# nucypher/TFHE.jl

Hardware: AMD Instinct MI355X
Metric: bootstrapped gates/sec (whole node), N=1024 (higher is better)
Workload: dtype int32 torus / f64 transform; 1 GPU; batch of 4096 independent gate_nand() bootstraps per GPU, tfhe_parameters_80 (n=500, N=1024, k=1, l=2, Bg=2^10, ks t=8, base 2^2); inputs=resident in HBM, launch=one process

## Files before the change

### tfhe.jl_amd/csrc/engine.hpp

```cpp
#pragma once
#include <hip/hip_runtime.h>

#include <algorithm>
#include <atomic>
#include <cstdarg>
#include <cstdio>
#include <cstring>
#include <new>
#include <string>
#include <thread>
#include <vector>

#include "../../include/tfhe_mi355x.h"
#include "experiment.hpp"
#include "br_core.hpp"

using namespace tfhe;

#include "kernels_blind_rotate.hpp"
#include "kernels_anyn.hpp"
#include "kernels_n512.hpp"
#include "kernels_keyswitch.hpp"

struct ErrBuf {
    char s[512] = {0};
    const char *c_str() const { return s; }
    void set(const char *msg) { snprintf(s, sizeof s, "%s", msg ? msg : ""); }
    ErrBuf &operator=(const char *msg) { set(msg); return *this; }
    void format(const char *fmt, ...) __attribute__((format(printf, 2, 3)))
    {
        va_list ap;
        va_start(ap, fmt);
        vsnprintf(s, sizeof s, fmt, ap);
        va_end(ap);
    }
};
extern thread_local ErrBuf g_create_error;

struct DevBuf {
    void *p = nullptr;
    size_t cap = 0;
    hipError_t reserve(size_t bytes)
    {
        if (bytes <= cap) return hipSuccess;
        if (p) (void)hipFree(p);
        p = nullptr; cap = 0;
        size_t want = bytes + bytes / 4 + 256;
        hipError_t e = hipMalloc(&p, want);
        if (e == hipSuccess) cap = want;
        return e;
    }
    void release() { if (p) (void)hipFree(p); p = nullptr; cap = 0; }
};

struct PairXfer {
    static constexpr int kSlots = 4;
    struct Slot {
        DevBuf out, idx_src;
        DevBuf in, idx_dst;
        int32_t *h_idx = nullptr; size_t h_idx_cap = 0;
        void *h_rows = nullptr; size_t h_rows_cap = 0;
        hipEvent_t ready = nullptr;
        hipEvent_t taken = nullptr;
        bool pending = false;
    } slot[kSlots];
    unsigned next = 0;
};

struct KsKey {
    int mode = 0;
    int parties = 1;
    int kN = 0;
    void *p = nullptr;
    size_t per_party = 0;
    int stride = 0;
    int wtiles = 0;
};
inline void release(KsKey &k)
{
    if (k.p) (void)hipFree(k.p);
    k = KsKey{};
}

struct tfhe_ctx {
    tfhe_params P{};
    int device = 0;
    ErrBuf err;
    std::vector<tfhe_ctx *> kids;
    std::vector<uint8_t> kid_ran;

    hipStream_t stream = nullptr;
    static constexpr int kTimingSlots = 33;
    hipEvent_t evring[kTimingSlots][4] = {};
    hipEvent_t *ev = evring[0];
    int64_t timed_calls = 0;
    hipEvent_t done_ev = nullptr;
    bool done_pending = false;
    bool timing_valid = false;
    bool own_pending = false;
    int64_t last_rotations = 0;
    std::string last_kernel;
    int ks_slices_large = 2;
    int ks_variant = 4;
    int64_t br_small = 1024;
    int br_prio_pct = 90;
    int br_general = 0;
    int br_split = 1;
    int timing_events = 1;
    int br_rt_l = 0;
    int64_t br_tiny = -2;

    cplx *d_tables = nullptr;
    Tables T{};
    Gadget g{};
    cplx *d_anyn_tab = nullptr;
    int br_anyn = 0;
    int anyn_spec = -1;
    bool anyn() const
    {
        if (br_anyn) return true;
        if (P.parties > 1) return P.N != kN || P.parties > 8 || P.bs_l > 8;
        if (n512()) return false;
        return (P.N != kN && P.N != 2048) || P.k > 4;
    }
    bool n512() const { return !br_anyn && P.parties == 1 && P.N == 512 && P.k == 1; }

    cplx *d_bk = nullptr;       size_t bk_polys = 0;
    KsKey ks;
    bool have_bk = false;
    bool have_ks() const { return ks.mode != 0 && ks.parties == 1; }
    cplx *d_mk_bk = nullptr;
    int mk_parties = 0;
    bool have_mk_bk = false;
    bool have_mk_ks() const { return ks.mode != 0 && ks.parties > 1; }

    int32_t *d_wires = nullptr; int64_t num_wires = 0;
    int wires_parties = 0;
    size_t wire_words() const { return wires_parties ? (size_t)wires_parties * P.n + 1 : (size_t)P.n + 1; }

    DevBuf bara, ext, map, io[4], diag, abar, mk_acc, spec;
    DevBuf tv, tv_index;
    DevBuf tv_bodies, tv_ext;
    cplx *d_tgsw = nullptr;        int64_t tgsw_count = 0;
    DevBuf lvl_ws[2], lvl_data, lvl_spec;
    cplx *d_mk_tgsw = nullptr;     int64_t mk_tgsw_count = 0;
    int32_t *d_mk_tgsw_party = nullptr;
    size_t diag_rows = 0;
    bool mk_force_general = false;
    int n2048_rw = 0;
    int mkg_rw = 0;
    int mkg_variant = 0;
    int mkg_acc = -1;
    int mk_rw = 0;
    bool measure_margin = false;
    int exact_domain = 2;
    double exact_bound_log2 = 0;
    double exact_margin = 0;
    tfhe_ctx *twin = nullptr;
    std::atomic<hipStream_t> twin_stream{nullptr};
    bool borrows_keys = false;
    bool slot_busy[2] = {false, false};
    std::atomic<std::thread::id> submit_thread{};
    uint32_t submits = 0;
    std::vector<std::vector<uint8_t>> wire_valid;
    std::vector<int32_t> wire_owner;
    std::vector<uint8_t> peer_ok;
    std::vector<struct PairXfer *> xfer;
    int level_exchange = 0;
    int64_t level_split_min = 4096;
    std::vector<int32_t> kid_tickets[2];
    int cu_count = 256;
    int w2_rw = 0;
    int n512_w2 = -1;
    int n512_rw = 0;
    int k2_w3 = -1;
    int k2_rw = 0;
    int v3_rw = 0;
    int64_t pipeline_min = 4096;
    bool last_call_two_streams = false;
    struct MapStage { void *h = nullptr; size_t cap = 0; hipEvent_t ev = nullptr; bool pending = false; };
    static constexpr int kMapStages = 4;
    MapStage map_stage[kMapStages];
    unsigned map_next = 0;
    MapStage *map_cur = &map_stage[0];
    void *h_map = nullptr;
// ... 200 lines not shown
```

### tfhe.jl_amd/csrc/engine_dispatch.hip

```cpp
#define TFHE_EMIT_KEYSWITCH_KERNELS
#include "engine.hpp"
#include "br_launch.hpp"

#include <map>
#include <mutex>
#include <functional>

int32_t ensure_dyn_lds(tfhe_ctx *c, const void *fn, size_t bytes, const char *what)
{
    static std::mutex mu;
    static std::map<std::pair<int, const void *>, size_t> have;
    std::lock_guard<std::mutex> lk(mu);
    size_t &cur = have[std::make_pair(c->device, fn)];
    if (cur >= bytes) return TFHE_OK;
    const hipError_t e = hipFuncSetAttribute(fn, hipFuncAttributeMaxDynamicSharedMemorySize, (int)bytes);
    if (e != hipSuccess) return c->set_err(TFHE_ERR_DEVICE, "hipFuncSetAttribute(%s, %zu bytes of LDS) failed: %s", what, bytes, hipGetErrorString(e));
    cur = bytes;
    return TFHE_OK;
}

int32_t prepare_diag(tfhe_ctx *c, size_t R, hipStream_t s, DiagArgs &d)
{
    d.margin_bits = nullptr; d.clk = nullptr; d.phase = nullptr;
    c->diag_rows = 0;
// ... 190 lines not shown
            if (best[i - n] + kK2RoundCost[n] < best[i]) { best[i] = best[i - n] + kK2RoundCost[n]; take[i] = n; }
    int tail = 0;
    double total = best[q];
    for (int t = 1; allow_w3 && t <= 2 && (size_t)t <= q; t++)
        if (best[q - t] + kK2W3RoundCost[t] < total) { total = best[q - t] + kK2W3RoundCost[t]; tail = t; }
    std::vector<int> rounds;
    for (size_t i = q - (size_t)tail; i > 0; i -= (size_t)take[i]) rounds.push_back(take[i]);
    std::sort(rounds.begin(), rounds.end(), std::greater<int>());
    std::vector<K2Seg> seg;
    size_t done = 0;
    for (size_t i = 0; i < rounds.size() && done < R;) {
        size_t j = i;
        while (j < rounds.size() && rounds[j] == rounds[i]) j++;
        const size_t want = (size_t)rounds[i] * (j - i) * cus;
        if ((j == rounds.size() && !tail) || done + want >= R) { seg.push_back({R - done, 0}); done = R; break; }
        seg.push_back({want, 0});
        done += want;
        i = j;
    }
    if (done < R) seg.push_back({R - done, 1});
    return seg;
}

int32_t launch_blind_rotate(tfhe_ctx *c, size_t R, int32_t mu, hipStream_t s, const TvPtrs *tv)
{
    if (tv && c->measure_margin) return c->set_err(TFHE_ERR_STATE, "bootstrap_tv: no DIAG instantiation of the TV kernels (measure_margin is on)");
    DiagArgs diag;
    int32_t rc = prepare_diag(c, R, s, diag);
    if (rc) return rc;
    alloc_checkpoint();
    std::vector<K2Seg> seg;
    const bool tuned_l = c->P.bs_l == 2 || c->P.bs_l == 3;
    if (c->anyn()) {
    } else if (c->br_split && !c->br_general && !c->measure_margin && c->P.N == kN && c->P.k == 2 && tuned_l && (c->k2_rw == 0 || c->k2_rw == 7) && c->k2_w3 != 1) {
        seg = k2_partition(R, (size_t)c->cu_count, c->k2_w3 < 0);
    } else if (c->br_split && !c->br_general && c->P.N == kN && c->P.k == 1 && c->br_small > 0) {
        const size_t resident = 8 * (size_t)c->cu_count;
        if (R > resident && R % resident > 0 && R % resident <= (size_t)c->br_small) seg = {{R - R % resident, -1}, {R % resident, -1}};
    }
    auto part = [&](size_t first, size_t count, int kind) {
        const int32_t r = launch_blind_rotate_part(c, first, count, mu, s, diag, kind, tv);
        if (!r && tv) c->last_kernel += "+tv";
        return r;
    };
    if (seg.empty()) return part(0, R, -1);
    if (seg.size() == 1) return part(0, R, seg[0].kind);
    std::string names;
    size_t first = 0;
    for (const K2Seg &sg : seg) {
        rc = part(first, sg.count, sg.kind);
        if (rc) return rc;
        if (names.empty() || names.substr(names.rfind(" + ") == std::string::npos ? 0 : names.rfind(" + ") + 3) != c->last_kernel)
            names += (names.empty() ? "" : " + ") + c->last_kernel;
        first += sg.count;
    }
    c->last_kernel = names;
    return TFHE_OK;
}

template <class A>
static A ks_args(const tfhe_ctx *c, const int32_t *e0, const int32_t *e1, const int32_t *dst, const int32_t *ext, int32_t *out)
{
    const int P = c->ks.parties, kN = c->ks.kN, n = c->P.n;
    A a{};
    a.ext = ext; a.e0 = e0; a.e1 = e1; a.dst = dst; a.out = out;
    a.n = n; a.kN = kN;
    a.in_stride = P * kN + 1; a.in_off = 0; a.in_b = P * kN; a.out_stride = P * n + 1; a.out_off = 0; a.out_b = P * n;
    return a;
}

int32_t launch_keyswitch(tfhe_ctx *c, size_t G, const int32_t *e0, const int32_t *e1, const int32_t *dst, const int32_t *ext, int32_t *out, hipStream_t s)
{
    const KsKey &K = c->ks;
    const int P = K.parties, kN = K.kN, n = c->P.n;
    if (K.mode == 4) {
        Ks4Args a = ks_args<Ks4Args>(c, e0, e1, dst, ext, out);
        a.G = (int)G; a.wtiles = K.wtiles;
        a.kslices = (P > 1 || kN % 512 != 0) ? 1 : (G <= 512 ? 16 : c->ks_slices_large);
        if (a.kslices > 1) {
            const Ks3Args i3 = ks_args<Ks3Args>(c, e0, e1, dst, ext, out);
            hipLaunchKernelGGL(ks3_init_kernel, dim3((unsigned)G), dim3(256), 0, s, i3);
        }
        a.Gpad = (int)((G + 63) / 64 * 64);
        HIP_TRY(c, c->abar.reserve((size_t)(kN / 4) * a.Gpad * 16));
        a.abar_t = (const i32x4 *)c->abar.p;
        for (int p = 0; p < P; p++) {
            a.in_off = p * kN; a.out_off = p * n; a.add_b = (p == 0);
            a.bmat = (const i32x4 *)K.p + (size_t)p * K.per_party;
            hipLaunchKernelGGL(ks4_digits_kernel, dim3((unsigned)(a.Gpad / 32), (unsigned)(kN / 128)), dim3(128), 0, s, a, (i32x4 *)c->abar.p);
            hipLaunchKernelGGL(keyswitch_kernel_v4, dim3((unsigned)((G + 255) / 256), (unsigned)K.wtiles, (unsigned)a.kslices), dim3(256), 0, s, a);
        }
    } else if (K.mode == 3) {
        Ks3Args a = ks_args<Ks3Args>(c, e0, e1, dst, ext, out);
        a.t = c->P.ks_t; a.log2_base = 2; a.stride = K.stride; a.G = (int)G;
        a.ksp = (const int32_t *)K.p;
        hipLaunchKernelGGL(ks3_init_kernel, dim3((unsigned)G), dim3(256), 0, s, a);
        const unsigned tiles = (unsigned)((G + KS3_G - 1) / KS3_G);
        for (int p = 0; p < P; p++) {
            a.in_off = p * kN; a.out_off = p * n;
            a.ksp = (const int32_t *)K.p + (size_t)p * K.per_party;
            hipLaunchKernelGGL(keyswitch_kernel_v3, dim3(tiles * KS3_SLICES, (unsigned)((K.stride + 511) / 512)), dim3(128), 0, s, a);
        }
    } else {
        KsArgs a = ks_args<KsArgs>(c, e0, e1, dst, ext, out);
        a.t = c->P.ks_t; a.log2_base = c->P.ks_log2_base;
        for (int p = 0; p < P; p++) {
            a.in_off = p * kN; a.out_off = p * n; a.add_b = (p == 0);
            a.ks = (const int32_t *)K.p + (size_t)p * K.per_party;
            hipLaunchKernelGGL(keyswitch_kernel, dim3((unsigned)G, (unsigned)((n + 1 + 256 * KS1_WPT - 1) / (256 * KS1_WPT))), dim3(256), 0, s, a);
        }
    }
    HIP_TRY(c, hipGetLastError());
    return TFHE_OK;
}
```

### tfhe.jl_amd/csrc/engine_keys.hip

```cpp
#define TFHE_EMIT_KEYPREP_KERNELS
#include "engine.hpp"
#include "kernels_keygen.hpp"

static int32_t check_key_source(tfhe_ctx *c, const void *p, const char *who)
{
    hipPointerAttribute_t at;
    const hipError_t e = hipPointerGetAttributes(&at, p);
    if (e != hipSuccess) { (void)hipGetLastError(); return TFHE_OK; }
    if (at.type == hipMemoryTypeDevice && at.device != c->device)
        return c->set_err(TFHE_ERR_DEVICE, "%s: the key buffer lives on device %d, this context on device %d: pass a host copy (peer access between GPUs is not assumed)",
                          who, at.device, c->device);
    return TFHE_OK;
}

void quiesce(tfhe_ctx *c)
{
    if (c->stream) (void)hipStreamSynchronize(c->stream);
    if (c->done_pending) { (void)hipEventSynchronize(c->done_ev); c->done_pending = false; }
    c->own_pending = false;
    if (c->twin && c->twin->stream) (void)hipStreamSynchronize(c->twin->stream);
    c->slot_busy[0] = c->slot_busy[1] = false;
    if (c->twin) {
        tfhe_ctx *t = c->twin;
        t->d_bk = nullptr; t->have_bk = false; t->ks = KsKey{};
// ... 39 lines not shown
        if (big && is_c128)
            hipLaunchKernelGGL(bk_permute_c128_kernel_n2048, dim3((unsigned)npolys), dim3(128), 0, c->stream, (const cplx *)d_in, c->d_bk);
        else if (big)
            hipLaunchKernelGGL(bk_prepare_kernel_n2048, dim3((unsigned)npolys), dim3(128), 0, c->stream, (const int32_t *)d_in, c->d_bk,
                               (const cplx *)(c->d_tables + kTableElems), c->T.tw2);
        else if (is_c128)
            hipLaunchKernelGGL(bk_permute_c128_kernel, dim3((unsigned)npolys), dim3(64), 0, c->stream, (const cplx *)d_in, c->d_bk);
        else
            hipLaunchKernelGGL(bk_prepare_kernel, dim3((unsigned)npolys), dim3(64), 0, c->stream, (const int32_t *)d_in, c->d_bk, c->T, 1.0 / kM);
        e = hipGetLastError();
    }
    if (e == hipSuccess) e = hipStreamSynchronize(c->stream);
    (void)hipFree(d_in);
    if (e != hipSuccess) return c->set_err(TFHE_ERR_DEVICE, "load_bootstrap_key: %s", hipGetErrorString(e));
    c->bk_polys = npolys;
    c->have_bk = true;
    return TFHE_OK;
}

int32_t tfhe_load_bootstrap_key_i32(tfhe_ctx *c, const int32_t *bk) try
{
    ENTER_CTX(c);
    if (!c) return TFHE_ERR_INVALID_ARG;
    return load_bk_common(c, bk, bk_poly_count(c->P) * (size_t)c->P.N * sizeof(int32_t), false);
}
ABI_CATCH(c, "tfhe_load_bootstrap_key_i32")

int32_t tfhe_load_bootstrap_key_c128(tfhe_ctx *c, const double *bk_spectra) try
{
    ENTER_CTX(c);
    if (!c) return TFHE_ERR_INVALID_ARG;
    return load_bk_common(c, bk_spectra, bk_poly_count(c->P) * (size_t)(c->P.N / 2) * sizeof(cplx), true);
}
ABI_CATCH(c, "tfhe_load_bootstrap_key_c128")

static size_t ks_row_count(const tfhe_params &p, int kN)
{
    return (size_t)kN * p.ks_t * ((1u << p.ks_log2_base) - 1);
}
static size_t ks_word_count(const tfhe_params &p)
{
    return ks_row_count(p, p.k * p.N) * (size_t)(p.n + 1);
}

static int pick_ks_mode(const tfhe_ctx *c, int kN)
{
    const bool ok4 = c->P.ks_log2_base == 2 && c->P.ks_t == 8 && kN % 128 == 0;
    const bool ok3 = c->P.ks_log2_base == 2 && c->P.ks_t % 4 == 0 && kN % KS3_SLICES == 0 && kN / KS3_SLICES <= 128;
    if (c->ks_variant == 4 && ok4) return 4;
    if (c->ks_variant >= 3 && ok3) return 3;
    return 1;
}

int32_t tfhe_load_keyswitch_key(tfhe_ctx *c, const int32_t *ks) try
{
    ENTER_CTX(c);
    if (!c) return TFHE_ERR_INVALID_ARG;
    if (!ks) return c->set_err(TFHE_ERR_INVALID_ARG, "load_keyswitch_key: NULL key pointer");
    if (c->P.parties != 1) return c->set_err(TFHE_ERR_STATE, "load_keyswitch_key: context is multi-key, use tfhe_mk_load_*");
    if (c->multi()) return fan_out(c, all_kids(c), [&](int k) { return tfhe_load_keyswitch_key(c->kids[(size_t)k], ks); });
    HIP_TRY(c, hipSetDevice(c->device));
    { const int32_t rcp = check_key_source(c, ks, "load_keyswitch_key"); if (rcp) return rcp; }
    const int kNn = c->P.k * c->P.N;
    const size_t n1 = (size_t)c->P.n + 1, rows = ks_row_count(c->P, kNn), bytes = rows * n1 * sizeof(int32_t);
    quiesce(c);
    release(c->ks);
    KsKey &K = c->ks;
    K.kN = kNn;
    int32_t *d_canon = nullptr;
    HIP_TRY(c, hipMalloc((void **)&d_canon, bytes));
    const int mode = pick_ks_mode(c, kNn);
    auto body = [&]() -> int32_t {
        HIP_TRY(c, hipMemcpyAsync(d_canon, ks, bytes, hipMemcpyDefault, c->stream));
        if (mode == 3) {
            const size_t stride = (n1 + 3) & ~(size_t)3;
            HIP_TRY(c, hipMalloc(&K.p, rows * stride * 4));
            HIP_TRY(c, hipMemsetAsync(K.p, 0, rows * stride * 4, c->stream));
            HIP_TRY(c, hipMemcpy2DAsync(K.p, stride * 4, d_canon, n1 * 4, n1 * 4, rows, hipMemcpyDeviceToDevice, c->stream));
            HIP_TRY(c, hipStreamSynchronize(c->stream));
            K.stride = (int)stride;
            K.per_party = rows * stride;
        } else if (mode == 4) {
            const int wtiles = (c->P.n + 1 + 31) / 32;
            const size_t frags = (size_t)kNn * wtiles * 4 * 64;
            HIP_TRY(c, hipMalloc(&K.p, frags * 16));
            hipLaunchKernelGGL(ks4_prepare_kernel, dim3((unsigned)((frags + 255) / 256)), dim3(256), 0, c->stream, (const int32_t *)d_canon,
                               (i32x4 *)K.p, c->P.n, kNn, wtiles);
            HIP_TRY(c, hipGetLastError());
            HIP_TRY(c, hipStreamSynchronize(c->stream));
            K.wtiles = wtiles;
            K.per_party = frags;
        }
        HIP_TRY(c, hipStreamSynchronize(c->stream));
        return TFHE_OK;
    };
    const int32_t rc = body();
    if (rc == TFHE_OK && mode == 1) { K.p = d_canon; K.per_party = rows * n1; }
    else (void)hipFree(d_canon);
    if (rc) return rc;
    K.mode = mode;
    return TFHE_OK;
}
ABI_CATCH(c, "tfhe_load_keyswitch_key")

int32_t tfhe_keygen_cloud_key(tfhe_ctx *c, const int32_t *lwe_key, const int32_t *tlwe_key, double bs_noise_stddev,
                              double ks_noise_stddev, const uint32_t *seed, int32_t *bk_out, int32_t *ks_out) try
{
    ENTER_CTX(c);
    if (!c) return TFHE_ERR_INVALID_ARG;
    if (!lwe_key || !tlwe_key || !seed) return c->set_err(TFHE_ERR_INVALID_ARG, "keygen_cloud_key: NULL key or seed pointer");
    if (c->P.parties != 1) return c->set_err(TFHE_ERR_STATE, "keygen_cloud_key: context is multi-key (use tfhe_mk_expand_load_bootstrap_key)");
    if (!(bs_noise_stddev >= 0.0) || !(ks_noise_stddev >= 0.0)) return c->set_err(TFHE_ERR_INVALID_ARG, "keygen_cloud_key: negative noise parameter");
    tfhe_ctx *g = c->multi() ? c->kids[0] : c;
    HIP_TRY(c, hipSetDevice(g->device));
    const tfhe_params &P = c->P;
    const size_t bk_words = bk_poly_count(P) * (size_t)P.N, ks_words = ks_word_count(P);
    const size_t Q = ks_words / (size_t)(P.n + 1), kN = (size_t)P.k * P.N;
    int32_t *d_lwe = nullptr, *d_tlwe = nullptr, *d_bk = nullptr, *d_ks = nullptr;
    double *d_noise = nullptr;
    auto cleanup = [&]() {
        if (d_lwe) (void)hipMemsetAsync(d_lwe, 0, (size_t)P.n * 4, g->stream);
        if (d_tlwe) (void)hipMemsetAsync(d_tlwe, 0, kN * 4, g->stream);
        if (d_noise) (void)hipMemsetAsync(d_noise, 0, (Q + 1) * sizeof(double), g->stream);
        (void)hipStreamSynchronize(g->stream);
        (void)hipFree(d_lwe); (void)hipFree(d_tlwe); (void)hipFree(d_bk); (void)hipFree(d_ks); (void)hipFree(d_noise);
    };
    auto body = [&]() -> int32_t {
        HIP_TRY(c, hipMalloc((void **)&d_lwe, (size_t)P.n * 4));
        HIP_TRY(c, hipMalloc((void **)&d_tlwe, kN * 4));
        HIP_TRY(c, hipMalloc((void **)&d_bk, bk_words * 4));
        HIP_TRY(c, hipMalloc((void **)&d_ks, ks_words * 4));
        HIP_TRY(c, hipMalloc((void **)&d_noise, (Q + 1) * sizeof(double)));
        HIP_TRY(c, hipMemcpyAsync(d_lwe, lwe_key, (size_t)P.n * 4, hipMemcpyHostToDevice, g->stream));
        HIP_TRY(c, hipMemcpyAsync(d_tlwe, tlwe_key, kN * 4, hipMemcpyHostToDevice, g->stream));
        keygen::Args A;
        A.lwe_key = d_lwe; A.tlwe_key = d_tlwe; A.bk = d_bk; A.ks = d_ks; A.ks_noise = d_noise; A.ks_mean = d_noise + Q;
        A.n = P.n; A.N = P.N; A.k = P.k; A.l = P.bs_l; A.beta = P.bs_log2_base; A.t = P.ks_t; A.ks_log2_base = P.ks_log2_base;
        A.bs_alpha = bs_noise_stddev; A.ks_alpha = ks_noise_stddev;
        for (int i = 0; i < 6; i++) A.seed.w[i] = seed[i];
        const size_t samples = (size_t)P.n * P.bs_l * (P.k + 1);
        const size_t lds = kN * 4 + (size_t)P.k * ((P.N + 31) / 32) * 4;
        hipLaunchKernelGGL(keygen::bk_kernel, dim3((unsigned)samples), dim3(256), lds, g->stream, A);
        hipLaunchKernelGGL(keygen::ks_noise_kernel, dim3((unsigned)((Q + 255) / 256)), dim3(256), 0, g->stream, A, Q);
        hipLaunchKernelGGL(keygen::ks_mean_kernel, dim3(1), dim3(256), 0, g->stream, A, Q);
        hipLaunchKernelGGL(keygen::ks_kernel, dim3((unsigned)((Q + 3) / 4)), dim3(256), 0, g->stream, A, Q);
        HIP_TRY(c, hipGetLastError());
        HIP_TRY(c, hipStreamSynchronize(g->stream));
        bool other_device = false;
        if (c->multi())
            for (const tfhe_ctx *k : c->kids) other_device = other_device || k->device != g->device;
        alloc_checkpoint();
        std::vector<int32_t> stage_bk, stage_ks;
        if (other_device && !bk_out) { stage_bk.resize(bk_words); bk_out = stage_bk.data(); }
        if (other_device && !ks_out) { stage_ks.resize(ks_words); ks_out = stage_ks.data(); }
        if (bk_out) HIP_TRY(c, hipMemcpyAsync(bk_out, d_bk, bk_words * 4, hipMemcpyDeviceToHost, g->stream));
        if (ks_out) HIP_TRY(c, hipMemcpyAsync(ks_out, d_ks, ks_words * 4, hipMemcpyDeviceToHost, g->stream));
        HIP_TRY(c, hipStreamSynchronize(g->stream));
        int32_t rc = tfhe_load_bootstrap_key_i32(c, other_device ? bk_out : d_bk);
        if (rc) return rc;
        return tfhe_load_keyswitch_key(c, other_device ? ks_out : d_ks);
    };
    auto guard = on_exit([&] { (void)hipSetDevice(g->device); cleanup(); });
    return body();
}
ABI_CATCH(c, "tfhe_keygen_cloud_key")

static int32_t launch_bk_prepare(tfhe_ctx *c, bool any, const int32_t *d_polys, cplx *d_out, size_t npolys, double scale_if_tuned, bool key_scale, hipStream_t s)
// ... 313 lines not shown
                                 const int32_t *d0, const int32_t *d1, const int32_t *f0, const int32_t *f1, int64_t S, int32_t *expanded_out) try
{
    ENTER_CTX(c);
    if (!c) return TFHE_ERR_INVALID_ARG;
    if (!pub_b || !c0 || !c1 || !d0 || !d1 || !f0 || !f1) return c->set_err(TFHE_ERR_INVALID_ARG, "mk_tgsw_expand_load: NULL argument");
    size_t per = 0;
    int32_t rc = mk_tgsw_check(c, "mk_tgsw_expand_load", party_of, S, parties, &per);
    if (rc) return rc;
    HIP_TRY(c, hipSetDevice(c->device));
    const int l = c->P.bs_l, P = parties;
    const size_t N = (size_t)c->P.N, M = N / 2 > 0 ? N / 2 : 1, lN = (size_t)l * N;
    alloc_checkpoint();
    std::vector<std::vector<int64_t>> of((size_t)P);
    for (int64_t s = 0; s < S; s++) of[(size_t)party_of[s]].push_back(s);
    size_t cap = 0;
    for (const auto &v : of) cap = std::max(cap, v.size());
    const size_t ndec = (size_t)(P - 1) * l * l;
    const double scratch = (6.0 * cap * lN + (double)ndec * N + (double)cap * per * N) * 4 + ((double)ndec + 2.0 * cap * l) * M * sizeof(cplx);
    MkExpandWork w;
    auto guard = on_exit([&] { w.release(); });
    return mk_tgsw_replace(c, "mk_tgsw_expand_load", party_of, S, per, scratch, [&](cplx *d_out) -> int32_t {
        int32_t rcp = mk_expand_alloc(c, w, P, cap);
        if (rcp) return rcp;
        hipStream_t s = c->stream;
        std::vector<int32_t> h_in(6 * cap * lN), h_key(expanded_out ? cap * per * N : 0);
        const int32_t *arr[6] = {c0, c1, d0, d1, f0, f1};
        for (int i = 0; i < P; i++) {
            const std::vector<int64_t> &mine = of[(size_t)i];
            const size_t cnt = mine.size();
            if (cnt == 0) continue;
            const int32_t *src[6];
            for (int a = 0; a < 6; a++) {
                int32_t *dst = h_in.data() + (size_t)a * cnt * lN;
                for (size_t j = 0; j < cnt; j++) memcpy(dst + j * lN, arr[a] + (size_t)mine[j] * lN, lN * 4);
                src[a] = dst;
            }
            rcp = mk_expand_party(c, w, true, P, i, (int)cnt, pub_b, src, s);
            if (rcp) return rcp;
            for (size_t j = 0; j < cnt; j++) {
                rcp = tgsw_prepare(c, w.d_key + j * per * N, d_out + (size_t)mine[j] * per * M, per, s);
                if (rcp) return rcp;
            }
            if (expanded_out) HIP_TRY(c, hipMemcpyAsync(h_key.data(), w.d_key, cnt * per * N * 4, hipMemcpyDeviceToHost, s));
            HIP_TRY(c, hipStreamSynchronize(s));
            if (expanded_out)
                for (size_t j = 0; j < cnt; j++) memcpy(expanded_out + (size_t)mine[j] * per * N, h_key.data() + j * per * N, per * N * 4);
        }
        return TFHE_OK;
    });
}
ABI_CATCH(c, "tfhe_mk_tgsw_expand_load")

int32_t tfhe_mk_load_keyswitch_key(tfhe_ctx *c, const int32_t *ks, int32_t parties) try
{
    ENTER_CTX(c);
    if (!c) return TFHE_ERR_INVALID_ARG;
    if (!ks) return c->set_err(TFHE_ERR_INVALID_ARG, "mk_load_keyswitch_key: NULL key pointer");
    if (parties < 2 || c->P.parties < parties)
        return c->set_err(TFHE_ERR_INVALID_ARG, "mk_load_keyswitch_key: parties must be at least 2 and not exceed the context's max_parties");
    if (c->multi()) return fan_out(c, all_kids(c), [&](int k) { return tfhe_mk_load_keyswitch_key(c->kids[(size_t)k], ks, parties); });
    HIP_TRY(c, hipSetDevice(c->device));
    const size_t n1 = (size_t)c->P.n + 1, stride = (n1 + 3) & ~(size_t)3;
    const size_t rows = ks_row_count(c->P, c->P.N);
    quiesce(c);
    release(c->ks);
    KsKey &K = c->ks;
    K.parties = parties;
    K.kN = c->P.N;
    const int mode = pick_ks_mode(c, c->P.N);
    if (mode == 1) {
        HIP_TRY(c, hipMalloc(&K.p, (size_t)parties * rows * n1 * 4));
        HIP_TRY(c, hipMemcpyAsync(K.p, ks, (size_t)parties * rows * n1 * 4, hipMemcpyHostToDevice, c->stream));
        HIP_TRY(c, hipStreamSynchronize(c->stream));
        K.per_party = rows * n1;
    } else if (mode == 3) {
        HIP_TRY(c, hipMalloc(&K.p, (size_t)parties * rows * stride * 4));
        HIP_TRY(c, hipMemsetAsync(K.p, 0, (size_t)parties * rows * stride * 4, c->stream));
        HIP_TRY(c, hipMemcpy2DAsync(K.p, stride * 4, ks, n1 * 4, n1 * 4, (size_t)parties * rows, hipMemcpyHostToDevice, c->stream));
        HIP_TRY(c, hipStreamSynchronize(c->stream));
        K.per_party = rows * stride;
        K.stride = (int)stride;
    } else {
        const int wtiles = (c->P.n + 1 + 31) / 32;
        const size_t frags = (size_t)c->P.N * wtiles * 4 * 64, words = rows * n1;
        int32_t *d_tmp = nullptr;
        HIP_TRY(c, hipMalloc((void **)&d_tmp, words * 4));
        auto body = [&]() -> int32_t {
            HIP_TRY(c, hipMalloc(&K.p, (size_t)parties * frags * 16));
            for (int p = 0; p < parties; p++) {
                HIP_TRY(c, hipMemcpyAsync(d_tmp, ks + (size_t)p * words, words * 4, hipMemcpyHostToDevice, c->stream));
                hipLaunchKernelGGL(ks4_prepare_kernel, dim3((unsigned)((frags + 255) / 256)), dim3(256), 0, c->stream, (const int32_t *)d_tmp,
                                   (i32x4 *)K.p + (size_t)p * frags, c->P.n, c->P.N, wtiles);
                HIP_TRY(c, hipGetLastError());
                HIP_TRY(c, hipStreamSynchronize(c->stream));
            }
            return TFHE_OK;
        };
        const int32_t rc = body();
        (void)hipFree(d_tmp);
        if (rc) return rc;
        K.per_party = frags;
        K.wtiles = wtiles;
    }
    K.mode = mode;
    return TFHE_OK;
}
ABI_CATCH(c, "tfhe_mk_load_keyswitch_key")
```

### tfhe.jl_amd/csrc/kernels_keyswitch.hpp

```cpp
#pragma once
#include <hip/hip_runtime.h>

#include "../../include/tfhe_mi355x.h"
#include "br_core.hpp"

using namespace tfhe;

struct KsArgs {
    const int32_t *ext;
    const int32_t *ks;
    const int32_t *e0;
    const int32_t *e1;
    const int32_t *dst;
    int32_t *out;
    int32_t n, kN, t, log2_base;
    int32_t in_stride, in_off, in_b, out_stride, out_off, out_b;
    int32_t add_b;
};

constexpr int KS1_WPT = 4;

#ifdef TFHE_EMIT_KEYSWITCH_KERNELS
__global__ __launch_bounds__(256) void keyswitch_kernel(KsArgs P)
{
    constexpr int WPT = KS1_WPT;
    const int g = blockIdx.x;
    const int tid = threadIdx.x;
    const int n1 = P.n + 1;
    const int w0 = blockIdx.y * (256 * WPT);
    const int32_t *x0 = P.ext + (size_t)P.e0[g] * P.in_stride;
    const int e1 = P.e1 ? P.e1[g] : -1;
    const int32_t *x1 = e1 >= 0 ? P.ext + (size_t)e1 * P.in_stride : nullptr;
    const int base1 = (1 << P.log2_base) - 1;
    const uint32_t prec_offset = 1u << (32 - (1 + P.log2_base * P.t));

    uint32_t accw[WPT];
#pragma unroll
    for (int u = 0; u < WPT; u++) accw[u] = 0;

    for (int i = 0; i < P.kN; i++) {
        uint32_t ai = (uint32_t)x0[P.in_off + i];
        if (x1) ai += (uint32_t)x1[P.in_off + i];
        const int32_t aibar = (int32_t)(ai + prec_offset);
        const int32_t *rows_i = P.ks + (size_t)i * P.t * base1 * n1;
        for (int j = 1; j <= P.t; j++) {
            const int d = (aibar >> (32 - j * P.log2_base)) & base1;
            if (d != 0) {
                const int32_t *row = rows_i + (size_t)((j - 1) * base1 + (d - 1)) * n1;
#pragma unroll
                for (int u = 0; u < WPT; u++) {
                    const int wd = w0 + tid + u * 256;
                    if (wd < n1) accw[u] -= (uint32_t)row[wd];
                }
            }
        }
    }
    const size_t og = P.dst ? (size_t)P.dst[g] : (size_t)g;
    int32_t *o = P.out + og * P.out_stride;
#pragma unroll
    for (int u = 0; u < WPT; u++) {
        const int wd = w0 + tid + u * 256;
        if (wd < P.n) {
            o[P.out_off + wd] = (int32_t)accw[u];
        } else if (wd == P.n) {
            uint32_t v = accw[u];
            if (P.add_b) {
                v += (uint32_t)x0[P.in_b];
                if (x1) v += (uint32_t)x1[P.in_b] + (1u << 29);
            } else {
                v += (uint32_t)o[P.out_b];
            }
            o[P.out_b] = (int32_t)v;
        }
    }
}
#endif

constexpr int KS3_G = 16;
constexpr int KS3_SLICES = 16;

struct Ks3Args {
    const int32_t *ext;
    const int32_t *ksp;
    const int32_t *e0, *e1, *dst;
    int32_t *out;
    int32_t n, kN, t, log2_base, stride, G;
    int32_t in_stride, in_off, in_b, out_stride, out_off, out_b;
// ... 26 lines not shown
    const int tid = threadIdx.x;
    const int lin = blockIdx.x;
    const int xcd = lin & 7;
    const int rest = lin >> 3;
    const int slice = xcd + 8 * (rest % (KS3_SLICES / 8));
    const int tile = rest / (KS3_SLICES / 8);
    const int wchunk = blockIdx.y;
    const int g0 = tile * G;
    const int slen = P.kN / KS3_SLICES;
    const int i0 = slice * slen;
    const int lb = P.log2_base, tl = P.t;
    const int base1 = (1 << lb) - 1;
    const uint32_t prec_offset = 1u << (32 - (1 + lb * tl));
    const int w0 = wchunk * 512 + tid * 4;
    const bool active = w0 < P.stride;
    const int wl = active ? w0 : 0;

    for (int idx = tid; idx < G * slen; idx += 128) {
        const int g = idx / slen, ii = idx % slen;
        const int gg = min(g0 + g, P.G - 1);
        uint32_t ai = (uint32_t)P.ext[(size_t)P.e0[gg] * P.in_stride + P.in_off + i0 + ii];
        const int e1 = P.e1 ? P.e1[gg] : -1;
        if (e1 >= 0) ai += (uint32_t)P.ext[(size_t)e1 * P.in_stride + P.in_off + i0 + ii];
        abar[g][ii] = (int32_t)(ai + prec_offset);
    }
    __syncthreads();

    u32x4 acc[G];
#pragma unroll
    for (int g = 0; g < G; g++) acc[g] = (u32x4)(0u);

    const size_t row_words = (size_t)P.stride;
    const int stages = slen * (tl / JH);
    auto load_stage = [&](int st, u32x4 (&r)[JH][3]) {
        const int ii = st / (tl / JH), jh = st % (tl / JH);
        const int32_t *rows = P.ksp + ((size_t)(i0 + ii) * tl + jh * JH) * base1 * row_words + wl;
#pragma unroll
        for (int j = 0; j < JH; j++)
#pragma unroll
            for (int h = 0; h < 3; h++) r[j][h] = *reinterpret_cast<const u32x4 *>(rows + (size_t)(j * 3 + h) * row_words);
    };
    auto compute_stage = [&](int st, const u32x4 (&r)[JH][3]) {
        const int ii = st / (tl / JH), jh = st % (tl / JH);
#pragma unroll
        for (int g = 0; g < G; g++) {
            const int a = __builtin_amdgcn_readfirstlane(abar[g][ii]);
#pragma unroll
            for (int j = 0; j < JH; j++) {
                const int pos = 32 - (jh * JH + j + 1) * lb;
                const uint32_t m0 = (uint32_t)((a << (31 - pos)) >> 31);
                const uint32_t m1 = (uint32_t)((a << (30 - pos)) >> 31);
                const u32x4 t = (r[j][2] & m1) | (r[j][0] & ~m1);
                const u32x4 u = r[j][1] & m1;
                acc[g] -= (t & m0) | (u & ~m0);
            }
        }
    };

    u32x4 ra[JH][3], rb[JH][3];
    load_stage(0, ra);
    for (int st = 0; st < stages; st += 2) {
        if (st + 1 < stages) load_stage(st + 1, rb);
        compute_stage(st, ra);
        if (st + 2 < stages) load_stage(st + 2, ra);
        if (st + 1 < stages) compute_stage(st + 1, rb);
    }

    if (!active) return;
#pragma unroll
    for (int g = 0; g < G; g++) {
        const int gg = g0 + g;
        if (gg >= P.G) break;
        const size_t og = P.dst ? (size_t)P.dst[gg] : (size_t)gg;
        int32_t *o = P.out + og * P.out_stride;
#pragma unroll
        for (int q = 0; q < 4; q++) {
            if (w0 + q < P.n) atomicAdd(reinterpret_cast<unsigned int *>(o + P.out_off + w0 + q), acc[g][q]);
            else if (w0 + q == P.n) atomicAdd(reinterpret_cast<unsigned int *>(o + P.out_b), acc[g][q]);
        }
    }
}
#endif

typedef int32_t i32x4 __attribute__((ext_vector_type(4)));
typedef int32_t i32x16 __attribute__((ext_vector_type(16)));

struct Ks4Args {
    const int32_t *ext;
    const i32x4 *bmat;
    const int32_t *e0, *e1, *dst;
    int32_t *out;
    int32_t n, kN, G, wtiles;
    int32_t in_stride, in_off, in_b, out_stride, out_off, out_b;
    int32_t add_b;
    const i32x4 *abar_t;
    int32_t Gpad;
    int32_t kslices;
};

__host__ __device__ inline int32_t signed_byte_plane(uint32_t v, int plane)
{
    int32_t s = 0;
    for (int p = 0; p <= plane; p++) {
        const uint32_t u = v & 255u;
        s = u >= 128u ? (int32_t)u - 256 : (int32_t)u;
        v = (v - (uint32_t)s) >> 8;
    }
    return s;
}

#ifdef TFHE_EMIT_KEYPREP_KERNELS
__global__ void ks4_prepare_kernel(const int32_t *__restrict__ ks, i32x4 *__restrict__ bmat, int n, int kN, int wtiles)
{
    const size_t idx = (size_t)blockIdx.x * blockDim.x + threadIdx.x;
    const size_t total = (size_t)kN * wtiles * 4 * 64;
    if (idx >= total) return;
    const int lane = (int)(idx & 63);
    const int plane = (int)((idx >> 6) & 3);
    const int wt = (int)((idx >> 8) % wtiles);
    const int i = (int)((idx >> 8) / wtiles);
    const int c = lane & 31, h = lane >> 5;
    const int w = wt * 32 + c;
    i32x4 frag;
    for (int q = 0; q < 4; q++) {
        const int j = 4 * h + q;
        uint32_t word = 0;
        for (int hh = 1; hh <= 3; hh++) {
            int32_t sb = 0;
            if (w <= n) sb = signed_byte_plane((uint32_t)ks[(((size_t)i * 8 + j) * 3 + (hh - 1)) * (n + 1) + w], plane);
            word |= ((uint32_t)sb & 255u) << (8 * hh);
        }
        frag[q] = (int32_t)word;
    }
    bmat[idx] = frag;
}
#endif

#ifdef TFHE_EMIT_KEYSWITCH_KERNELS
__global__ __launch_bounds__(128) void ks4_digits_kernel(Ks4Args P, i32x4 *__restrict__ abar_t)
{
    __shared__ uint32_t tile[32][129];
    const int tid = threadIdx.x;
    const int g0 = blockIdx.x * 32, i0 = blockIdx.y * 128;
    for (int g = 0; g < 32; g++) {
        const int gg = min(g0 + g, P.G - 1);
        const int32_t *r0 = P.ext + (size_t)P.e0[gg] * P.in_stride + P.in_off;
        const int e1 = P.e1 ? P.e1[gg] : -1;
        uint32_t v = (uint32_t)r0[i0 + tid];
        if (e1 >= 0) v += (uint32_t)P.ext[(size_t)e1 * P.in_stride + P.in_off + i0 + tid];
        tile[g][tid] = v + (1u << 15);
    }
    __syncthreads();
    for (int k = tid; k < 32 * 32; k += 128) {
        const int q = k >> 5, g = k & 31;
        i32x4 o;
#pragma unroll
        for (int u = 0; u < 4; u++) o[u] = (int32_t)tile[g][4 * q + u];
        abar_t[(size_t)(i0 / 4 + q) * P.Gpad + g0 + g] = o;
    }
}

__global__ __launch_bounds__(256, 2) void keyswitch_kernel_v4(Ks4Args P)
{
    constexpr int MT = 2;
    __shared__ i32x4 bst[2][4][4][64];
    const int lane = threadIdx.x & 63, wave = threadIdx.x >> 6;
    const int c = lane & 31, h = lane >> 5;
    const int wt = blockIdx.y;
    const int gbase = (blockIdx.x * 4 + wave) * (32 * MT);
    const bool wave_active = gbase < P.G;

    const i32x4 *ap[MT];
#pragma unroll
    for (int mt = 0; mt < MT; mt++) ap[mt] = P.abar_t + min(gbase + mt * 32 + c, P.Gpad - 1);

    i32x16 acc[MT][4];
#pragma unroll
    for (int mt = 0; mt < MT; mt++)
#pragma unroll
        for (int pl = 0; pl < 4; pl++)
#pragma unroll
            for (int r = 0; r < 16; r++) acc[mt][pl][r] = 0;

    const size_t bstep = (size_t)P.wtiles * 4 * 64;
    const int i_begin = (int)blockIdx.z * (P.kN / P.kslices), i_end = i_begin + P.kN / P.kslices;
    const i32x4 *bp = P.bmat + (size_t)i_begin * bstep + ((size_t)wt * 4 + wave) * 64 + lane;
    const int stages = (i_end - i_begin) / 4;
    i32x4 pre[4];
#pragma unroll
    for (int ii = 0; ii < 4; ii++) bst[0][ii][wave][lane] = bp[(size_t)ii * bstep];

    i32x4 a_cur[MT], a_nxt[MT];
    auto load_a = [&](int i4, i32x4 (&a)[MT]) {
#pragma unroll
        for (int mt = 0; mt < MT; mt++) a[mt] = ap[mt][(size_t)(i4 >> 2) * P.Gpad];
    };
    load_a(i_begin, a_cur);

    for (int st = 0; st < stages; st++) {
        const bool more = st + 1 < stages;
        if (more) {
#pragma unroll
            for (int ii = 0; ii < 4; ii++) pre[ii] = bp[(size_t)(4 * (st + 1) + ii) * bstep];
            load_a(i_begin + 4 * (st + 1), a_nxt);
        }
        __syncthreads();
        if (wave_active) {
#pragma unroll
            for (int ii = 0; ii < 4; ii++) {
                i32x4 afrag[MT];
#pragma unroll
                for (int mt = 0; mt < MT; mt++)
#pragma unroll
                    for (int q = 0; q < 4; q++) {
                        const uint32_t d8 = ((uint32_t)a_cur[mt][ii] >> (27 - 2 * (4 * h + q))) & 24u;
                        afrag[mt][q] = (int32_t)(1u << d8);
                    }
#pragma unroll
                for (int pl = 0; pl < 4; pl++) {
                    const i32x4 bfrag = bst[st & 1][ii][pl][lane];
#pragma unroll
                    for (int mt = 0; mt < MT; mt++)
                        acc[mt][pl] = __builtin_amdgcn_mfma_i32_32x32x32_i8(afrag[mt], bfrag, acc[mt][pl], 0, 0, 0);
                }
            }
        }
        if (more) {
#pragma unroll
            for (int ii = 0; ii < 4; ii++) bst[(st + 1) & 1][ii][wave][lane] = pre[ii];
#pragma unroll
            for (int mt = 0; mt < MT; mt++) a_cur[mt] = a_nxt[mt];
        }
    }
    if (!wave_active) return;

    const int w = wt * 32 + c;
    if (w > P.n) return;
#pragma unroll
    for (int mt = 0; mt < MT; mt++)
#pragma unroll
        for (int r = 0; r < 16; r++) {
            const int gg = gbase + mt * 32 + (r & 3) + 8 * (r >> 2) + 4 * h;
            if (gg >= P.G) continue;
            uint32_t sum = (uint32_t)acc[mt][0][r] + ((uint32_t)acc[mt][1][r] << 8) + ((uint32_t)acc[mt][2][r] << 16) +
                           ((uint32_t)acc[mt][3][r] << 24);
            const size_t og = P.dst ? (size_t)P.dst[gg] : (size_t)gg;
            int32_t *o = P.out + og * P.out_stride;
            if (P.kslices > 1) {
                atomicAdd(reinterpret_cast<unsigned int *>(o + (w < P.n ? P.out_off + w : P.out_b)), 0u - sum);
            } else if (w < P.n) {
                o[P.out_off + w] = (int32_t)(0u - sum);
            } else {
                if (P.add_b) {
                    uint32_t b = (uint32_t)P.ext[(size_t)P.e0[gg] * P.in_stride + P.in_b];
                    const int e1 = P.e1 ? P.e1[gg] : -1;
                    if (e1 >= 0) b += (uint32_t)P.ext[(size_t)e1 * P.in_stride + P.in_b] + (1u << 29);
                    o[P.out_b] = (int32_t)(b - sum);
                } else {
                    o[P.out_b] = (int32_t)((uint32_t)o[P.out_b] - sum);
                }
            }
        }
}
#endif
```

Measured before the change: 355,600 gates/s.

## Restructure MFMA keyswitch with digit-slot key layout, XCD-aware grid and deeper prefetch

```diff
diff --git a/tfhe.jl_amd/csrc/engine.hpp b/tfhe.jl_amd/csrc/engine.hpp
--- a/tfhe.jl_amd/csrc/engine.hpp
+++ b/tfhe.jl_amd/csrc/engine.hpp
@@ -100,7 +100,7 @@
     bool own_pending = false;
     int64_t last_rotations = 0;
     std::string last_kernel;
-    int ks_slices_large = 2;
+    int ks_slices_large = 1;
     int ks_variant = 4;
     int64_t br_small = 1024;
     int br_prio_pct = 90;
diff --git a/tfhe.jl_amd/csrc/engine_dispatch.hip b/tfhe.jl_amd/csrc/engine_dispatch.hip
--- a/tfhe.jl_amd/csrc/engine_dispatch.hip
+++ b/tfhe.jl_amd/csrc/engine_dispatch.hip
@@ -296,13 +296,14 @@
             hipLaunchKernelGGL(ks3_init_kernel, dim3((unsigned)G), dim3(256), 0, s, i3);
         }
         a.Gpad = (int)((G + 63) / 64 * 64);
+        a.sblocks = (int)((G + KS4_BLOCK_G - 1) / KS4_BLOCK_G);
         HIP_TRY(c, c->abar.reserve((size_t)(kN / 4) * a.Gpad * 16));
         a.abar_t = (const i32x4 *)c->abar.p;
         for (int p = 0; p < P; p++) {
             a.in_off = p * kN; a.out_off = p * n; a.add_b = (p == 0);
             a.bmat = (const i32x4 *)K.p + (size_t)p * K.per_party;
             hipLaunchKernelGGL(ks4_digits_kernel, dim3((unsigned)(a.Gpad / 32), (unsigned)(kN / 128)), dim3(128), 0, s, a, (i32x4 *)c->abar.p);
-            hipLaunchKernelGGL(keyswitch_kernel_v4, dim3((unsigned)((G + 255) / 256), (unsigned)K.wtiles, (unsigned)a.kslices), dim3(256), 0, s, a);
+            hipLaunchKernelGGL(keyswitch_kernel_v4, dim3(ks4_grid(K.wtiles * a.kslices, a.sblocks)), dim3(64 * KS4_WAVES), 0, s, a);
         }
     } else if (K.mode == 3) {
         Ks3Args a = ks_args<Ks3Args>(c, e0, e1, dst, ext, out);
diff --git a/tfhe.jl_amd/csrc/engine_keys.hip b/tfhe.jl_amd/csrc/engine_keys.hip
--- a/tfhe.jl_amd/csrc/engine_keys.hip
+++ b/tfhe.jl_amd/csrc/engine_keys.hip
@@ -145,7 +145,7 @@
             K.per_party = rows * stride;
         } else if (mode == 4) {
             const int wtiles = (c->P.n + 1 + 31) / 32;
-            const size_t frags = (size_t)kNn * wtiles * 4 * 64;
+            const size_t frags = ks4_frag_count(kNn, wtiles);
             HIP_TRY(c, hipMalloc(&K.p, frags * 16));
             hipLaunchKernelGGL(ks4_prepare_kernel, dim3((unsigned)((frags + 255) / 256)), dim3(256), 0, c->stream, (const int32_t *)d_canon,
                                (i32x4 *)K.p, c->P.n, kNn, wtiles);
@@ -625,7 +625,7 @@
         K.stride = (int)stride;
     } else {
         const int wtiles = (c->P.n + 1 + 31) / 32;
-        const size_t frags = (size_t)c->P.N * wtiles * 4 * 64, words = rows * n1;
+        const size_t frags = ks4_frag_count(c->P.N, wtiles), words = rows * n1;
         int32_t *d_tmp = nullptr;
         HIP_TRY(c, hipMalloc((void **)&d_tmp, words * 4));
         auto body = [&]() -> int32_t {
diff --git a/tfhe.jl_amd/csrc/kernels_keyswitch.hpp b/tfhe.jl_amd/csrc/kernels_keyswitch.hpp
--- a/tfhe.jl_amd/csrc/kernels_keyswitch.hpp
+++ b/tfhe.jl_amd/csrc/kernels_keyswitch.hpp
@@ -3,6 +3,7 @@
 
 #include "../../include/tfhe_mi355x.h"
 #include "br_core.hpp"
+#include "ks_slots.hpp"
 
 using namespace tfhe;
 
@@ -195,8 +196,17 @@
 }
 #endif
 
+typedef int32_t i32x2 __attribute__((ext_vector_type(2)));
 typedef int32_t i32x4 __attribute__((ext_vector_type(4)));
 typedef int32_t i32x16 __attribute__((ext_vector_type(16)));
+
+constexpr int KS4_WAVES = 8;
+constexpr int KS4_BLOCK_G = 32 * KS4_WAVES;
+constexpr int KS4_STAGE_GROUPS = 2;
+constexpr int KS4_STAGE_WORDS = KS4_GROUP * KS4_STAGE_GROUPS;
+constexpr int KS4_STAGE_FRAGS = KS4_FRAGS * KS4_STAGE_GROUPS;
+constexpr int KS4_WAVE_FRAGS = KS4_STAGE_FRAGS / KS4_WAVES;
+static_assert(KS4_STAGE_FRAGS % KS4_WAVES == 0, "every wave stages the same number of fragments");
 
 struct Ks4Args {
     const int32_t *ext;
@@ -209,40 +219,23 @@
     const i32x4 *abar_t;
     int32_t Gpad;
     int32_t kslices;
+    int32_t sblocks;
 };
-
-__host__ __device__ inline int32_t signed_byte_plane(uint32_t v, int plane)
-{
-    int32_t s = 0;
-    for (int p = 0; p <= plane; p++) {
-        const uint32_t u = v & 255u;
-        s = u >= 128u ? (int32_t)u - 256 : (int32_t)u;
-        v = (v - (uint32_t)s) >> 8;
-    }
-    return s;
-}
 
 #ifdef TFHE_EMIT_KEYPREP_KERNELS
 __global__ void ks4_prepare_kernel(const int32_t *__restrict__ ks, i32x4 *__restrict__ bmat, int n, int kN, int wtiles)
 {
     const size_t idx = (size_t)blockIdx.x * blockDim.x + threadIdx.x;
-    const size_t total = (size_t)kN * wtiles * 4 * 64;
-    if (idx >= total) return;
+    if (idx >= ks4_frag_count(kN, wtiles)) return;
     const int lane = (int)(idx & 63);
-    const int plane = (int)((idx >> 6) & 3);
-    const int wt = (int)((idx >> 8) % wtiles);
-    const int i = (int)((idx >> 8) / wtiles);
+    const int f = (int)((idx >> 6) % KS4_FRAGS), m = f >> 2, plane = f & 3;
+    const size_t gw = (idx >> 6) / KS4_FRAGS;
+    const int wt = (int)(gw % wtiles), g = (int)(gw / wtiles);
     const int c = lane & 31, h = lane >> 5;
-    const int w = wt * 32 + c;
     i32x4 frag;
     for (int q = 0; q < 4; q++) {
-        const int j = 4 * h + q;
         uint32_t word = 0;
-        for (int hh = 1; hh <= 3; hh++) {
-            int32_t sb = 0;
-            if (w <= n) sb = signed_byte_plane((uint32_t)ks[(((size_t)i * 8 + j) * 3 + (hh - 1)) * (n + 1) + w], plane);
-            word |= ((uint32_t)sb & 255u) << (8 * hh);
-        }
+        for (int b = 4 * q; b < 4 * q + 4; b++) word |= ((uint32_t)ks4_b_byte(ks, n, g, m, plane, h, b, wt * 32 + c) & 255u) << (8 * (b & 3));
         frag[q] = (int32_t)word;
     }
     bmat[idx] = frag;
@@ -273,106 +266,122 @@
     }
 }
 
-__global__ __launch_bounds__(256, 2) void keyswitch_kernel_v4(Ks4Args P)
-{
-    constexpr int MT = 2;
-    __shared__ i32x4 bst[2][4][4][64];
+__global__ __launch_bounds__(64 * KS4_WAVES) void keyswitch_kernel_v4(Ks4Args P)
+{
+    constexpr int SG = KS4_STAGE_GROUPS, WF = KS4_WAVE_FRAGS;
+    __shared__ i32x4 bst[2][KS4_STAGE_FRAGS][64];
+    int unit, sblock;
+    ks4_block_unit((int)blockIdx.x, P.sblocks, unit, sblock);
+    if (unit >= P.wtiles * P.kslices) return;
+    const int wt = unit % P.wtiles, slice = unit / P.wtiles;
     const int lane = threadIdx.x & 63, wave = threadIdx.x >> 6;
     const int c = lane & 31, h = lane >> 5;
-    const int wt = blockIdx.y;
-    const int gbase = (blockIdx.x * 4 + wave) * (32 * MT);
+    const int gbase = (sblock * KS4_WAVES + wave) * 32;
     const bool wave_active = gbase < P.G;
 
-    const i32x4 *ap[MT];
-#pragma unroll
-    for (int mt = 0; mt < MT; mt++) ap[mt] = P.abar_t + min(gbase + mt * 32 + c, P.Gpad - 1);
-
-    i32x16 acc[MT][4];
-#pragma unroll
-    for (int mt = 0; mt < MT; mt++)
-#pragma unroll
-        for (int pl = 0; pl < 4; pl++)
-#pragma unroll
-            for (int r = 0; r < 16; r++) acc[mt][pl][r] = 0;
-
-    const size_t bstep = (size_t)P.wtiles * 4 * 64;
-    const int i_begin = (int)blockIdx.z * (P.kN / P.kslices), i_end = i_begin + P.kN / P.kslices;
-    const i32x4 *bp = P.bmat + (size_t)i_begin * bstep + ((size_t)wt * 4 + wave) * 64 + lane;
-    const int stages = (i_end - i_begin) / 4;
-    i32x4 pre[4];
-#pragma unroll
-    for (int ii = 0; ii < 4; ii++) bst[0][ii][wave][lane] = bp[(size_t)ii * bstep];
-
-    i32x4 a_cur[MT], a_nxt[MT];
-    auto load_a = [&](int i4, i32x4 (&a)[MT]) {
-#pragma unroll
-        for (int mt = 0; mt < MT; mt++) a[mt] = ap[mt][(size_t)(i4 >> 2) * P.Gpad];
-    };
-    load_a(i_begin, a_cur);
-
-    for (int st = 0; st < stages; st++) {
-        const bool more = st + 1 < stages;
-        if (more) {
-#pragma unroll
-            for (int ii = 0; ii < 4; ii++) pre[ii] = bp[(size_t)(4 * (st + 1) + ii) * bstep];
-            load_a(i_begin + 4 * (st + 1), a_nxt);
-        }
+    i32x16 acc[4];
+#pragma unroll
+    for (int pl = 0; pl < 4; pl++)
+#pragma unroll
+        for (int r = 0; r < 16; r++) acc[pl][r] = 0;
+
+    const int slice_words = P.kN / P.kslices;
+    const int g_begin = slice * slice_words / KS4_GROUP;
+    const int stages = slice_words / KS4_STAGE_WORDS;
+    const size_t gstep = (size_t)P.wtiles * KS4_FRAGS * 64;
+    const i32x4 *bp[WF];
+#pragma unroll
+    for (int u = 0; u < WF; u++) {
+        const int f = wave * WF + u;
+        bp[u] = P.bmat + (size_t)(g_begin + f / KS4_FRAGS) * gstep + ((size_t)wt * KS4_FRAGS + f % KS4_FRAGS) * 64 + lane;
+    }
+    const i32x2 *ap = reinterpret_cast<const i32x2 *>(P.abar_t + (size_t)g_begin * P.Gpad + min(gbase + c, P.Gpad - 1)) + h;
+    const size_t astep = (size_t)P.Gpad * 2;
+
+    struct Pre { i32x4 b[WF]; i32x2 a[SG]; };
+    auto fetch = [&](int st, Pre &x) {
+        const size_t s = (size_t)min(st, stages - 1) * SG;
+#pragma unroll
+        for (int u = 0; u < WF; u++) x.b[u] = bp[u][s * gstep];
+#pragma unroll
+        for (int gi = 0; gi < SG; gi++) x.a[gi] = ap[(s + gi) * astep];
+    };
+    auto stage_out = [&](int st, const Pre &x) {
+#pragma unroll
+        for (int u = 0; u < WF; u++) bst[st & 1][wave * WF + u][lane] = x.b[u];
+    };
+    auto compute = [&](int st, const i32x2 (&a)[SG]) {
+        constexpr int UNITS = SG * KS4_STEPS;
+        i32x4 bf[2][4];
+        auto read_unit = [&](int u, i32x4 (&b)[4]) {
+#pragma unroll
+            for (int pl = 0; pl < 4; pl++) b[pl] = bst[st & 1][u * 4 + pl][lane];
+        };
+        read_unit(0, bf[0]);
+        i32x4 afrag[SG][KS4_STEPS];
+#pragma unroll
+        for (int gi = 0; gi < SG; gi++) {
+            uint32_t f0[KS4_STEPS][2], f1[KS4_STEPS][2];
+            ks4_a_word((uint32_t)a[gi][0], f0);
+            ks4_a_word((uint32_t)a[gi][1], f1);
+#pragma unroll
+            for (int m = 0; m < KS4_STEPS; m++) afrag[gi][m] = i32x4{(int32_t)f0[m][0], (int32_t)f0[m][1], (int32_t)f1[m][0], (int32_t)f1[m][1]};
+        }
+#pragma unroll
+        for (int u = 0; u < UNITS; u++) {
+            if (u + 1 < UNITS) read_unit(u + 1, bf[(u + 1) & 1]);
+            __builtin_amdgcn_sched_barrier(0);
+#pragma unroll
+            for (int pl = 0; pl < 4; pl++)
+                acc[pl] = __builtin_amdgcn_mfma_i32_32x32x32_i8(afrag[u / KS4_STEPS][u % KS4_STEPS], bf[u & 1][pl], acc[pl], 0, 0, 0);
+            __builtin_amdgcn_sched_barrier(0);
+        }
+    };
+    i32x2 a_cur[SG];
+    auto step = [&](int st, Pre &cur, Pre &nxt) {
+        fetch(st + 2, nxt);
         __syncthreads();
-        if (wave_active) {
-#pragma unroll
-            for (int ii = 0; ii < 4; ii++) {
-                i32x4 afrag[MT];
-#pragma unroll
-                for (int mt = 0; mt < MT; mt++)
-#pragma unroll
-                    for (int q = 0; q < 4; q++) {
-                        const uint32_t d8 = ((uint32_t)a_cur[mt][ii] >> (27 - 2 * (4 * h + q))) & 24u;
-                        afrag[mt][q] = (int32_t)(1u << d8);
-                    }
-#pragma unroll
-                for (int pl = 0; pl < 4; pl++) {
-                    const i32x4 bfrag = bst[st & 1][ii][pl][lane];
-#pragma unroll
-                    for (int mt = 0; mt < MT; mt++)
-                        acc[mt][pl] = __builtin_amdgcn_mfma_i32_32x32x32_i8(afrag[mt], bfrag, acc[mt][pl], 0, 0, 0);
-                }
-            }
-        }
-        if (more) {
-#pragma unroll
-            for (int ii = 0; ii < 4; ii++) bst[(st + 1) & 1][ii][wave][lane] = pre[ii];
-#pragma unroll
-            for (int mt = 0; mt < MT; mt++) a_cur[mt] = a_nxt[mt];
-        }
+        if (wave_active) compute(st, a_cur);
+        stage_out(st + 1, cur);
+#pragma unroll
+        for (int gi = 0; gi < SG; gi++) a_cur[gi] = cur.a[gi];
+    };
+
+    Pre p0, p1;
+    fetch(0, p0);
+    fetch(1, p1);
+    stage_out(0, p0);
+#pragma unroll
+    for (int gi = 0; gi < SG; gi++) a_cur[gi] = p0.a[gi];
+    for (int st = 0; st < stages; st += 2) {
+        step(st, p1, p0);
+        step(st + 1, p0, p1);
     }
     if (!wave_active) return;
 
     const int w = wt * 32 + c;
     if (w > P.n) return;
 #pragma unroll
-    for (int mt = 0; mt < MT; mt++)
-#pragma unroll
-        for (int r = 0; r < 16; r++) {
-            const int gg = gbase + mt * 32 + (r & 3) + 8 * (r >> 2) + 4 * h;
-            if (gg >= P.G) continue;
-            uint32_t sum = (uint32_t)acc[mt][0][r] + ((uint32_t)acc[mt][1][r] << 8) + ((uint32_t)acc[mt][2][r] << 16) +
-                           ((uint32_t)acc[mt][3][r] << 24);
-            const size_t og = P.dst ? (size_t)P.dst[gg] : (size_t)gg;
-            int32_t *o = P.out + og * P.out_stride;
-            if (P.kslices > 1) {
-                atomicAdd(reinterpret_cast<unsigned int *>(o + (w < P.n ? P.out_off + w : P.out_b)), 0u - sum);
-            } else if (w < P.n) {
-                o[P.out_off + w] = (int32_t)(0u - sum);
+    for (int r = 0; r < 16; r++) {
+        const int gg = gbase + (r & 3) + 8 * (r >> 2) + 4 * h;
+        if (gg >= P.G) continue;
+        uint32_t sum = (uint32_t)acc[0][r] + ((uint32_t)acc[1][r] << 8) + ((uint32_t)acc[2][r] << 16) + ((uint32_t)acc[3][r] << 24);
+        const size_t og = P.dst ? (size_t)P.dst[gg] : (size_t)gg;
+        int32_t *o = P.out + og * P.out_stride;
+        if (P.kslices > 1) {
+            atomicAdd(reinterpret_cast<unsigned int *>(o + (w < P.n ? P.out_off + w : P.out_b)), 0u - sum);
+        } else if (w < P.n) {
+            o[P.out_off + w] = (int32_t)(0u - sum);
+        } else {
+            if (P.add_b) {
+                uint32_t b = (uint32_t)P.ext[(size_t)P.e0[gg] * P.in_stride + P.in_b];
+                const int e1 = P.e1 ? P.e1[gg] : -1;
+                if (e1 >= 0) b += (uint32_t)P.ext[(size_t)e1 * P.in_stride + P.in_b] + (1u << 29);
+                o[P.out_b] = (int32_t)(b - sum);
             } else {
-                if (P.add_b) {
-                    uint32_t b = (uint32_t)P.ext[(size_t)P.e0[gg] * P.in_stride + P.in_b];
-                    const int e1 = P.e1 ? P.e1[gg] : -1;
-                    if (e1 >= 0) b += (uint32_t)P.ext[(size_t)e1 * P.in_stride + P.in_b] + (1u << 29);
-                    o[P.out_b] = (int32_t)(b - sum);
-                } else {
-                    o[P.out_b] = (int32_t)((uint32_t)o[P.out_b] - sum);
-                }
+                o[P.out_b] = (int32_t)((uint32_t)o[P.out_b] - sum);
             }
         }
-}
-#endif
+    }
+}
+#endif
diff --git a/tfhe.jl_amd/csrc/ks_slots.hpp b/tfhe.jl_amd/csrc/ks_slots.hpp
--- /dev/null
+++ b/tfhe.jl_amd/csrc/ks_slots.hpp
@@ -0,0 +1,79 @@
+#pragma once
+#include <stddef.h>
+#include <stdint.h>
+
+#ifndef TFHE_HD
+#if defined(__HIPCC__)
+#include <hip/hip_runtime.h>
+#define TFHE_HD __host__ __device__ __forceinline__
+#else
+#define TFHE_HD inline
+#endif
+#endif
+
+namespace tfhe {
+
+constexpr int KS4_GROUP = 4;
+constexpr int KS4_STEPS = 3;
+constexpr int KS4_FRAGS = KS4_STEPS * 4;
+
+TFHE_HD int32_t signed_byte_plane(uint32_t v, int plane)
+{
+    int32_t s = 0;
+    for (int p = 0; p <= plane; p++) {
+        const uint32_t u = v & 255u;
+        s = u >= 128u ? (int32_t)u - 256 : (int32_t)u;
+        v = (v - (uint32_t)s) >> 8;
+    }
+    return s;
+}
+
+TFHE_HD int ks4_slot_word(int h, int b) { return 2 * h + (b >> 3); }
+TFHE_HD int ks4_slot_digit(int b) { return (b & 7) ^ 3; }
+TFHE_HD int ks4_word_half(int ii) { return ii >> 1; }
+TFHE_HD int ks4_word_digit_byte(int ii, int j) { return 8 * (ii & 1) + (j ^ 3); }
+
+TFHE_HD size_t ks4_frag_index(int g, int wt, int wtiles, int m, int pl, int lane)
+{
+    return (((size_t)g * wtiles + wt) * KS4_FRAGS + (m * 4 + pl)) * 64 + lane;
+}
+TFHE_HD size_t ks4_frag_count(int kN_words, int wtiles) { return (size_t)(kN_words / KS4_GROUP) * wtiles * KS4_FRAGS * 64; }
+
+TFHE_HD int32_t ks4_b_byte(const int32_t *ks, int n, int g, int m, int pl, int h, int b, int w)
+{
+    if (w > n) return 0;
+    const size_t i = (size_t)g * KS4_GROUP + ks4_slot_word(h, b);
+    return signed_byte_plane((uint32_t)ks[((i * 8 + ks4_slot_digit(b)) * 3 + m) * (size_t)(n + 1) + w], pl);
+}
+
+TFHE_HD uint32_t ks4_spread4(uint32_t y)
+{
+    const uint32_t z = (y | (y << 12)) & 0x000F000Fu;
+    return z | (z << 6);
+}
+TFHE_HD void ks4_flags(uint32_t z, uint32_t (&f)[KS4_STEPS])
+{
+    const uint32_t lo = z & 0x01010101u, hi = (z >> 1) & 0x01010101u;
+    f[2] = lo & hi;
+    f[0] = lo ^ f[2];
+    f[1] = hi ^ f[2];
+}
+TFHE_HD void ks4_a_word(uint32_t abar, uint32_t (&f)[KS4_STEPS][2])
+{
+    uint32_t t[KS4_STEPS];
+    ks4_flags(ks4_spread4(abar >> 24), t);
+    for (int m = 0; m < KS4_STEPS; m++) f[m][0] = t[m];
+    ks4_flags(ks4_spread4((abar >> 16) & 255u), t);
+    for (int m = 0; m < KS4_STEPS; m++) f[m][1] = t[m];
+}
+
+constexpr int KS4_XCDS = 8;
+TFHE_HD unsigned ks4_grid(int units, int sblocks) { return (unsigned)((units + KS4_XCDS - 1) / KS4_XCDS * KS4_XCDS * sblocks); }
+TFHE_HD void ks4_block_unit(int id, int sblocks, int &unit, int &sblock)
+{
+    const int xcd = id % KS4_XCDS, rest = id / KS4_XCDS;
+    unit = (rest / sblocks) * KS4_XCDS + xcd;
+    sblock = rest % sblocks;
+}
+
+}
```

Result: faster. 359,500 gates/s (median of 5 runs) (+1.1%).
